# JosefAlbers/Phi-3-Vision-MLX

Measured on AMD Instinct MI355X. Metric: decode tokens/sec through generate()'s loop (reference-defined; bare graph replays: device_rate) + prefill ms, Phi-3-Vision bf16 1-image VQA, higher is better.
Workload: dtype bf16; 1 GPU; Phi-3-Vision single 336x336 image VQA (BASELINE configs[1]); 17 crops, 2509 image tokens + 22 text tokens, prompt 2531, B=1 per GPU, greedy, EOS suppressed; parallelism=batch-sharded replicas x1, batch_per_gpu=1, tiny=False

## Files before the change

include/p3v.h:

```cpp
#ifndef P3V_H
#define P3V_H
#include <stdint.h>

#ifdef __cplusplus
extern "C" {
#endif

#define P3V_VERSION 600
#define P3V_OK 0
#define P3V_ERR_ARG (-22)
#define P3V_ERR_LAUNCH (-5)
#define P3V_ERR_UNSUPPORTED (-95)
#define P3V_ERR_HIP (-14)

typedef struct {
  int cu_count, lds_per_cu, wave_size, clock_khz, mem_clock_khz, mem_bus_bits;
  int64_t hbm_bytes;
  char arch[32];
} p3v_props_t;

int p3v_version(void);
int p3v_device_props(int device, p3v_props_t* out );
const char* p3v_strerror(int code);

// ... 38 lines not shown
int p3v_gemm_rows_slices(int M, int N, int K, int epilogue);

typedef struct {
  const uint16_t* x;
  const uint16_t* W;
  void* out;
  const uint16_t* resid;
  const uint16_t* norm_w;
  float norm_eps;
  int M, N, K;
  int epilogue;
} p3v_gemv_args_t;
int p3v_gemv(const p3v_gemv_args_t* args , void* stream);

typedef struct {
  const uint16_t* x; const uint8_t* W; const float* w_scale; void* out;
  const uint16_t* resid; const uint16_t* norm_w;
  float norm_eps;
  int M, N, K;
  int epilogue;
} p3v_gemv_fp8_args_t;
int p3v_gemv_fp8(const p3v_gemv_fp8_args_t* args , void* stream);
int p3v_dequant_fp8(const uint8_t* w8, const float* w_scale, uint16_t* out_bf16, int rows, int K, void* stream);

typedef struct {
  const uint8_t* A; const float* a_scale; const uint8_t* W; const float* w_scale;
  uint16_t* out; const uint16_t* resid;
  int M, N, K, lda, ldw, ldo, epilogue;
} p3v_gemm_fp8_args_t;
int p3v_gemm_fp8(const p3v_gemm_fp8_args_t* args , void* stream);
int p3v_quant_fp8_rows(const uint16_t* x, const uint16_t* norm_w , float eps, uint8_t* q, float* scale,
                       int rows, int K, void* stream);

int p3v_rope_table(const float* pos, const float* inv_freq, float scale, float* cos_out, float* sin_out,
                   int n_pos, int half_dim, void* stream);

int p3v_rope_kv_append(const uint16_t* qkv, const float* cos_t, const float* sin_t,
                       uint16_t* q_out, uint16_t* k_dst, uint16_t* v_dst,
                       int B, int L, int n_heads, int n_kv, int hd,
                       int past, const int32_t* d_past, int dst_t, int dst_off_is_past,
                       int tab_t, int tab_div, float q_scale, void* stream);

int p3v_gemm_resid_norm(const p3v_gemm_args_t* gemm , const uint16_t* norm_w, float eps, uint16_t* normed, void* stream);

typedef struct {
  const float* cos_t; const float* sin_t;
// ... 104 lines not shown
                     int epilogue, const uint16_t* resid, uint16_t* out, int M, int N, int K, int r_max, int n_slots,
                     void* stream);

int p3v_add_i32(int32_t* x, int n, int delta, void* stream);
int p3v_store_token(const int32_t* tok, int32_t* history, const int32_t* d_step, int32_t* tok_next,
                    int B, int max_steps, void* stream);
int p3v_step_begin(const int32_t* tok, const uint16_t* table, uint16_t* x_out, const float* cos_t, const float* sin_t,
                   const int32_t* d_past, float* cos_out, float* sin_out, int B, int hidden, int vocab, int tab_t,
                   int half_dim, int32_t* zero_buf ,
                   int n_zero, void* stream);
int p3v_step_end(const uint16_t* logits, int32_t* next_tok, int32_t* tok, int32_t* history, int32_t* d_step,
                 int32_t* d_past, int32_t* ticket, int B, int n, int max_steps, void* stream);

#define P3V_GEMV_STEP_MAX_WG 1024
#define P3V_GEMV_STEP_WS_BYTES (P3V_GEMV_STEP_MAX_WG * 8 + 9 * 128)
typedef struct {
  const int32_t* tok; const uint16_t* embed_table; int vocab; uint16_t* x_out;
  const float* cos_t; const float* sin_t; float* cos_out; float* sin_out; int tab_t, half_dim;
  int32_t* next_tok; int32_t* tok_out; int32_t* history; int32_t* d_step; int32_t* ticket; float* amax_ws; int max_steps;
  int32_t* d_past;
} p3v_gemv_step_t;
int p3v_gemv_step(const p3v_gemv_args_t* args , const p3v_gemv_step_t* step , void* stream);
int p3v_gemv_fp8_step(const p3v_gemv_fp8_args_t* args , const p3v_gemv_step_t* step , void* stream);
int p3v_gemv_q4_step(const p3v_gemv_q4_args_t* args , const p3v_gemv_step_t* step , void* stream);

typedef struct {
  float temperature;
  int32_t top_k;
  float top_p;
  uint32_t seed_lo, seed_hi;
  int32_t counter;
} p3v_sample_row_t;
int p3v_sample(const uint16_t* logits, int64_t row_stride, p3v_sample_row_t* rows_params, int32_t* out, int rows, int n,
               void* stream);
int p3v_sample_step_end(const uint16_t* logits, p3v_sample_row_t* rows_params, int32_t* next_tok, int32_t* tok,
                        int32_t* history, int32_t* d_step, int32_t* d_past, int32_t* ticket, int B, int n, int max_steps,
                        void* stream);

#define P3V_LOGPROBS_MAX 8
typedef struct {
  int32_t token;
  float   logprob;
  int32_t rank;
  int32_t n_top;
  int32_t top_id[P3V_LOGPROBS_MAX];
  float   top_logprob[P3V_LOGPROBS_MAX];
// ... 53 lines not shown
```

phi-3-vision-mlx_amd/_lib.py:

```python
import ctypes as C
import os

_HERE = os.path.dirname(os.path.abspath(__file__))
LIB_PATH = os.environ.get("P3V_LIB") or os.path.join(_HERE, "libp3v.so")

P3V_OK = 0
(EPI_NONE, EPI_BIAS, EPI_BIAS_QGELU, EPI_BIAS_GELU, EPI_BIAS_RESID_F32, EPI_RESID_BF16, EPI_SILU_MUL, EPI_PATCH,
 EPI_F32) = range(9)
DECODE_MAX_L = 16

vp, i32, i64, f32 = C.c_void_p, C.c_int, C.c_int64, C.c_float


class Props(C.Structure):
    _fields_ = [("cu_count", i32), ("lds_per_cu", i32), ("wave_size", i32), ("clock_khz", i32),
                ("mem_clock_khz", i32), ("mem_bus_bits", i32), ("hbm_bytes", i64), ("arch", C.c_char * 32)]


class GemmArgs(C.Structure):
    _fields_ = [("A", vp), ("W", vp), ("out", vp), ("bias", vp), ("resid", vp), ("pos", vp),
                ("M", i32), ("N", i32), ("K", i32), ("lda", i32), ("ldw", i32), ("ldo", i32),
                ("epilogue", i32), ("patches_per_img", i32), ("ws", vp), ("ws_bytes", i64)]


# ... 1 lines not shown
    _fields_ = [("cos_t", vp), ("sin_t", vp), ("q_out", vp), ("k_dst", vp), ("v_dst", vp),
                ("B", i32), ("L", i32), ("n_heads", i32), ("n_kv", i32), ("hd", i32),
                ("past", i32), ("dst_t", i32), ("dst_off_is_past", i32), ("tab_t", i32), ("tab_div", i32), ("q_scale", f32)]


class GemvArgs(C.Structure):
    _fields_ = [("x", vp), ("W", vp), ("out", vp), ("resid", vp), ("norm_w", vp), ("norm_eps", f32),
                ("M", i32), ("N", i32), ("K", i32), ("epilogue", i32)]


class GemvStep(C.Structure):
    _fields_ = [("tok", vp), ("embed_table", vp), ("vocab", i32), ("x_out", vp),
                ("cos_t", vp), ("sin_t", vp), ("cos_out", vp), ("sin_out", vp), ("tab_t", i32), ("half_dim", i32),
                ("next_tok", vp), ("tok_out", vp), ("history", vp), ("d_step", vp), ("ticket", vp), ("amax_ws", vp), ("max_steps", i32),
                ("d_past", vp)]


GEMV_STEP_WS_BYTES = 1024 * 8 + 9 * 128


class GemvF8Args(C.Structure):
    _fields_ = [("x", vp), ("W", vp), ("w_scale", vp), ("out", vp), ("resid", vp), ("norm_w", vp), ("norm_eps", f32),
                ("M", i32), ("N", i32), ("K", i32), ("epilogue", i32)]


class GemmF8Args(C.Structure):
    _fields_ = [("A", vp), ("a_scale", vp), ("W", vp), ("w_scale", vp), ("out", vp), ("resid", vp),
                ("M", i32), ("N", i32), ("K", i32), ("lda", i32), ("ldw", i32), ("ldo", i32), ("epilogue", i32)]


class AttnArgs(C.Structure):
    _fields_ = [("q", vp), ("k_past", vp), ("v_past", vp), ("k_new", vp), ("v_new", vp), ("out", vp),
                ("pad_len", vp), ("d_past", vp), ("ws", vp),
                ("B", i32), ("L", i32), ("n_heads", i32), ("n_kv", i32), ("hd", i32),
                ("past", i32), ("past_t", i32), ("past_div", i32), ("new_t", i32), ("pad_div", i32),
                ("causal", i32), ("scale", f32), ("n_split", i32), ("new_is_cache", i32), ("q_prescaled", i32)]


class GemvQ4Args(C.Structure):
    _fields_ = [("x", vp), ("W", vp), ("sb", vp), ("out", vp), ("resid", vp), ("norm_w", vp), ("norm_eps", f32),
                ("M", i32), ("N", i32), ("K", i32), ("epilogue", i32)]


class AttnDecArgs(C.Structure):
    _fields_ = [("qkv", vp), ("cos_t", vp), ("sin_t", vp), ("k_cache", vp), ("v_cache", vp), ("out", vp),
                ("pad_len", vp), ("d_past", vp), ("ws", vp),
# ... 43 lines not shown
SPEC_REC_INTS, SPEC_CTL_INTS, SPEC_NGRAM_CAP = 18, 8, 8
SPEC_CTL_N, SPEC_CTL_NDRAFT, SPEC_CTL_FORCED, SPEC_CTL_REPLAY, SPEC_CTL_NLIMIT, SPEC_CTL_ACC = range(6)
KV_COPY_MAX_JOBS = 4
LORA_SLICE_K, LORA_MAX_RANK = 256, 64
SAMPLE_MAX_N, SAMPLE_MAX_ROWS = 32768, 1024
SIGNATURES = {
    "p3v_version": (i32, []),
    "p3v_device_props": (i32, [i32, C.POINTER(Props)]),
    "p3v_strerror": (C.c_char_p, [i32]),
    "p3v_set_tuning": (i32, [C.c_char_p, i32]),
    "p3v_get_tuning": (i32, [C.c_char_p, C.POINTER(i32)]),
    "p3v_embed_gather": (i32, [vp, vp, vp, i32, i32, i32, vp]),
    "p3v_rmsnorm": (i32, [vp, vp, vp, i32, i32, f32, vp]),
    "p3v_layernorm": (i32, [vp, vp, vp, vp, i32, i32, i32, f32, vp]),
    "p3v_gemm": (i32, [C.POINTER(GemmArgs), vp]),
    "p3v_gemm_ws_bytes": (i64, [i32, i32, i32, i32]),
    "p3v_gemm_rows_slices": (i32, [i32, i32, i32, i32]),
    "p3v_gemv": (i32, [C.POINTER(GemvArgs), vp]),
    "p3v_gemv_step": (i32, [C.POINTER(GemvArgs), C.POINTER(GemvStep), vp]),
    "p3v_gemv_fp8_step": (i32, [C.POINTER(GemvF8Args), C.POINTER(GemvStep), vp]),
    "p3v_gemv_q4_step": (i32, [C.POINTER(GemvQ4Args), C.POINTER(GemvStep), vp]),
    "p3v_gemv_fp8": (i32, [C.POINTER(GemvF8Args), vp]),
    "p3v_dequant_fp8": (i32, [vp, vp, vp, i32, i32, vp]),
    "p3v_gemm_fp8": (i32, [C.POINTER(GemmF8Args), vp]),
    "p3v_quant_fp8_rows": (i32, [vp, vp, f32, vp, vp, i32, i32, vp]),
    "p3v_rope_table": (i32, [vp, vp, f32, vp, vp, i32, i32, vp]),
    "p3v_rope_kv_append": (i32, [vp, vp, vp, vp, vp, vp, i32, i32, i32, i32, i32, i32, vp, i32, i32, i32, i32, f32, vp]),
    "p3v_attention": (i32, [C.POINTER(AttnArgs), vp]),
    "p3v_attention_decode": (i32, [C.POINTER(AttnDecArgs), vp]),
    "p3v_attention_decode_can_fuse_oproj": (i32, [i32, i32, i32, i32, i32, i32, i32, i32]),
    "p3v_attention_decode_fused_role": (i32, [i32, i32, i32, i32, i32, C.POINTER(i32)]),
    "p3v_kv_quantize": (i32, [vp, vp, vp, vp, vp, vp, i32, i32, i32, i32, i32, i32, vp]),
    "p3v_kv_dequantize": (i32, [vp, vp, vp, vp, vp, vp, i32, i32, i32, i32, i32, vp]),
    "p3v_gemm_qkv": (i32, [vp, vp, vp]),
    "p3v_gemm_resid_norm": (i32, [C.POINTER(GemmArgs), vp, f32, vp, vp]),
    "p3v_kv_quantize_mlx4": (i32, [vp, vp, vp, vp, vp, vp, i32, i32, i32, i32, vp, vp, vp, i32, i32, i32, i32, i32, vp]),
    "p3v_attention_decode_q8": (i32, [C.POINTER(AttnDecQ8Args), vp]),
    "p3v_attention_decode_q8_can_fuse_oproj": (i32, [i32, i32, i32, i32, i32, i32, i32, i32]),
    "p3v_stage_rope": (i32, [vp, vp, i32, vp, vp, vp, i32, i32, i32, i32, vp]),
    "p3v_attention_ws_bytes": (i64, [i32, i32, i32, i32, i32]),
    "p3v_im2col_patches": (i32, [vp, vp, i32, i32, i32, i32, vp]),
    "p3v_clip_cls_rows": (i32, [vp, vp, vp, i32, i32, i32, vp]),
    "p3v_hd_merge": (i32, [vp, vp, vp, vp, i32, i32, i32, i32, vp]),
    "p3v_argmax": (i32, [vp, vp, i32, i32, i64, vp]),
    "p3v_log_softmax": (i32, [vp, vp, i32, i32, vp]),
    "p3v_topk": (i32, [vp, vp, i32, i32, i32, i64, vp]),
# ... 58 lines not shown
```

phi-3-vision-mlx_amd/model.py:

```python
import math
import copy
import os

import numpy as np
import torch

from . import ops
from .config import head_dim, is_vision, rope_scaling_factor
from .weights import Q4Weight, mlx_quantize, q4_repack
from .ops import (BF16, EPI_BIAS, EPI_BIAS_GELU, EPI_BIAS_QGELU, EPI_BIAS_RESID_F32, EPI_NONE, EPI_PATCH,
                  EPI_RESID_BF16, EPI_SILU_MUL, F32, I32)

import functools
import weakref


def _on_device(fn):
    @functools.wraps(fn)
    def wrapped(self, *a, **kw):
        with torch.cuda.device(self.device):
            return fn(self, *a, **kw)
    return wrapped


# ... 123 lines not shown
        self.w8 = {}
        self._rope_tables = {}
        self._vit_graphs, self._vit_seen = {}, {}
        self.adapters = {}
        self._lora_tmp = {}
        self._lora_flat = None
        self.adapter_names = []
        self._bank = {}
        self._bank_keep = []
        self._rows_cur = None
        self.serving = os.environ.get("P3V_SHARED_GPU", "0") == "1"
        self.epoch = 0
        self._prefill_graphs = {}
        self._prefill_seen = {}
        self._states = weakref.WeakSet()
        self.fp8_act = bool(getattr(cfg, "fp8_activations", True)) and os.environ.get("P3V_FP8_PREFILL", "mfma") != "dequant"
        if getattr(cfg, "quantized_fp8", False):
            self._quantize_decoder_fp8()
        if getattr(cfg, "quantized_int4", False):
            self._quantize_decoder_q4()
        if self.w4 and not hasattr(self, "_deq"):
            n_max = max(v[0].shape[0] * v[0].shape[1] * 8 for v in self.w4.values())
            self._deq = torch.empty(n_max, dtype=BF16, device=self.device)
        if self.vision:
            self._prep_vision()

    def _quantize_decoder_fp8(self):
        names = [k for k in self.w if k == "lm_head.weight" or (k.startswith("model.layers.") and k.endswith("_proj.weight"))]
        for k in names:
            self.w8[k] = ops.quantize_fp8_rows(self.w.pop(k))
        n_max = max(v[0].shape[0] * v[0].shape[1] for v in self.w8.values())
        self._deq = torch.empty(n_max, dtype=BF16, device=self.device)

    def set_adapters(self, adapters):
        if adapters and self._bank:
            raise ValueError("this model carries an adapter bank (set_adapter_bank): detach it before set_adapters -- one or the other")
        self._set_adapters(adapters)

    @_on_device
    def _set_adapters(self, adapters):
        for k, (a, b, _) in adapters.items():
            shape = self._weight_shape(k)
            if tuple(a.shape[:1]) != (shape[1],) or tuple(b.shape[1:]) != (shape[0],):
                raise ValueError(f"LoRA shapes {tuple(a.shape)} x {tuple(b.shape)} do not fit {k} {tuple(shape)}")
        self.adapters = {k: (a.to(self.device, F32).contiguous(), b.to(self.device, F32).contiguous(), float(s))
                         for k, (a, b, s) in adapters.items()}
        self.epoch += 1
        for st in list(self._states):
            st.graphs.clear()
        self._lora_tmp, self._lora_flat = {}, None
        self._prefill_graphs.clear()

    def _weight_shape(self, k):
        if k in self.w:
            return tuple(self.w[k].shape)
# ... 95 lines not shown
        for k in names:
            self.w4[k] = tuple(t.to(self.device) for t in q4_repack(*mlx_quantize(self.w.pop(k))))

    def _proj(self, x, key, epilogue=EPI_NONE, resid=None, norm_w=None, out=None, h=None):
        ad = self.adapters.get(key)
        if ad is None:
            bk = self._bank.get(key) if self._bank else None
            if bk is not None:
                return self._proj_bank(x, key, bk[0], bk[1], epilogue, resid, norm_w, out, h)
            return self._proj_frozen(x, key, epilogue, resid, norm_w, out, h)
        a, b, scale = ad
        M, K, N, r = x.shape[0], x.shape[1], b.shape[1], a.shape[1]
        hbuf, y, t = self._lora_scratch(M, [("h", (M, K), BF16), ("y", (M, N), BF16), ("t", (M, r), F32)])
        if norm_w is not None:
            x = ops.rmsnorm(x, norm_w, self.cfg.rms_norm_eps, out=hbuf)
        self._proj_frozen(x, key, EPI_NONE, None, None, y, None)
        ops.lora_down(x, a, out=t)
        return ops.lora_up(y, t, b, scale, epilogue, resid=resid, out=out)

    def _proj_frozen(self, x, key, epilogue=EPI_NONE, resid=None, norm_w=None, out=None, h=None):
        eps = self.cfg.rms_norm_eps
        M, K = x.shape
        q, q4 = self.w8.get(key), self.w4.get(key)
        skinny = M <= 8 or (M <= ops.GEMV_MAX_M and K % 512 == 0)
        if skinny and M > 8 and q is None and q4 is None and K % 64 == 0 and self.w[key].shape[0] % 64 == 0:
            skinny = False
        if q4 is not None and M == 1 and K in (3072, 8192):
            return ops.gemv_q4(x, q4[0], q4[1], epilogue, resid=resid, norm_w=norm_w, norm_eps=eps, out=out)
        if (q4 is not None and 2 <= M <= 16 and K in (3072, 8192) and os.environ.get("P3V_Q4_ROWS", "1") != "0"
                and (q4[0].shape[0] // (2 if epilogue == EPI_SILU_MUL else 1)) % 16 == 0):
            if norm_w is not None and (M > 8 or os.environ.get("P3V_Q4_ROWS8_NORM", "1") == "0"):
                x, norm_w = ops.rmsnorm(x, norm_w, eps, out=h), None
            return ops.gemv_q4(x, q4[0], q4[1], epilogue, resid=resid, norm_w=norm_w, norm_eps=eps, out=out)
        if q is not None and skinny and K in (3072, 8192):
            return ops.gemv_fp8(x, q[0], q[1], epilogue, resid=resid, norm_w=norm_w, norm_eps=eps, out=out)
        if q is not None and not skinny and self.fp8_act and ops.gemm_fp8_ok(M, q[0].shape[0], K, epilogue):
            a8, sa = ops.quant_fp8_rows(x, norm_w, eps)
            return ops.gemm_fp8(a8, sa, q[0], q[1], epilogue, resid=resid, out=out)
        if q4 is not None:
            w = ops.dequant_q4(q4[0], q4[1], out=self._deq[:q4[0].numel() * 8].view(q4[0].shape[0], q4[0].shape[1] * 8))
        elif q is not None:
            w = ops.dequant_fp8(q[0], q[1], out=self._deq[:q[0].numel()].view(q[0].shape))
        else:
            w = self.w[key]
        if skinny:
            return ops.gemv(x, w, epilogue, resid=resid, norm_w=norm_w, norm_eps=eps, out=out)
# ... 383 lines not shown
        if (st.quantized or mlx4) and n_beam > 1:
            raise NotImplementedError("Beam Search is not yet compatible with Quantized Cache")
        mlx4_first = mlx4 and past == 0 and st.mlx4_tokens == 0 and L <= st.k4.shape[3]
        if n_beam > 1:
            Lp = (L + 7) // 8 * 8
            k_new = torch.empty((B, nkv, Lp, hd), dtype=BF16, device=self.device)
            v_new = torch.zeros((B, nkv, hd, Lp), dtype=BF16, device=self.device)
        normed_in = False
        for i in range(cfg.num_hidden_layers):
            p = f"model.layers.{i}."
            fused_qkv = False
            k_w = p + "self_attn.qkv_proj.weight"
            if (not decode and n_beam == 1 and k_w in w and k_w not in self.adapters and k_w not in self._bank and not mlx4_first
                    and (M >= 1024 or M <= 256) and os.environ.get("P3V_QKV_FUSE", "1") != "0"):
                kd, vd = (st.k_tmp, st.v_tmp) if st.quantized else (st.k[i], st.v[i])
                if not (st.quantized and past > 0 and not st.fresh_rows):
                    hn = h if normed_in else ops.rmsnorm(x, w[p + "input_layernorm.weight"], eps, out=h)
                    normed_in = True
                    fused_qkv = ops.gemm_qkv(hn, w[k_w], st.cos, st.sin, q, kd, vd, B, L, nh, nkv, hd, past, st.Tp, True, st.T, 1,
                                             q_scale=scale * ops.Q_PRESCALE)
            if i == 0 and step_begin is not None:
                sb = step_begin
                w_fold = w.get(k_w) if k_w in w else (self.w8.get(k_w) or self.w4.get(k_w))
                if not (w_fold is not None and k_w not in self.adapters and k_w not in self._bank and os.environ.get("P3V_STEP_FOLD", "1") != "0"
                        and ops.gemv_step_begin(sb["tok"], sb["table"], x, st.cos, st.sin, d_past, sb["cos_o"], sb["sin_o"],
                                                w_fold, w[p + "input_layernorm.weight"], eps, qkv)):
                    ops.step_begin(sb["tok"], sb["table"], x, st.cos, st.sin, d_past, sb["cos_o"], sb["sin_o"])
                    self._proj(x, k_w, norm_w=w[p + "input_layernorm.weight"], out=qkv, h=h)
            elif not fused_qkv:
                if normed_in:
                    self._proj(h, p + "self_attn.qkv_proj.weight", out=qkv)
                else:
                    self._proj(x, p + "self_attn.qkv_proj.weight", norm_w=w[p + "input_layernorm.weight"], out=qkv, h=h)
            o_i = o
            if fuse_o:
                o_i, o_other = (bufs["o_f"], bufs["o_f2"]) if i % 2 == 0 else (bufs["o_f2"], bufs["o_f"])
            if st.quantized:
                if decode:
                    kw_o = {}
                    if fuse_o:
                        w8o = self.w8[p + "self_attn.o_proj.weight"]
                        kw_o = dict(o_proj_w8=w8o[0], o_proj_scale=w8o[1], o_proj_x=x, o_rearm=o_other)
                    ops.attention_decode_q8(qkv, rc, rs, rb, st.k8[i], st.v8[i], st.ks[i], st.vs[i], o_i, B, L, nh, nkv,
                                            hd, scale, past, st.Tp, ws, n_split, pad_len=st.pad_len, d_past=d_past,
                                            merge_in_launch=attn_merge, **kw_o)
                else:
# ... 66 lines not shown
    def _build_decode_graph(self, st):
        cfg, B, dev = self.cfg, st.B, self.device
        g = dict(tok=torch.zeros((B,), dtype=I32, device=dev), d_past=torch.zeros((1,), dtype=I32, device=dev),
                 d_step=torch.zeros((1,), dtype=I32, device=dev),
                 history=torch.zeros((B, max(1, st.max_tokens) + 1), dtype=I32).pin_memory(),
                 x=torch.empty((B, cfg.hidden_size), dtype=BF16, device=dev),
                 logits=torch.empty((B, cfg.vocab_size), dtype=BF16, device=dev),
                 next_tok=torch.zeros((B,), dtype=I32, device=dev), ticket=torch.zeros((1,), dtype=I32, device=dev))
        g["bufs"] = self._plan(st, B, 1, fuse_o=not st.slots, captured=True)
        g["amax_ws"] = torch.zeros((ops.L.GEMV_STEP_WS_BYTES // 4,), dtype=F32, device=dev)
        g["d_past"].fill_(st.offset)
        g["gemm_ws"] = {}
        g["graph"] = self._capture(lambda: self._decode_step(st, g), g["gemm_ws"])
        g["d_step"].zero_()
        return g

    def _decode_step(self, st, g, sampled=False, logprobs=False):
        cfg, w, bufs, head = self.cfg, self.w, g["bufs"], "lm_head.weight"
        self._layers(g["x"], st, st.B, 1, 0, 1, bufs=bufs, d_past=g["d_past"],
                     step_begin=dict(tok=g["tok"], table=w["model.embed_tokens.weight"], cos_o=bufs["rope_cos"], sin_o=bufs["rope_sin"]))
        end = (g["next_tok"], g["tok"], g["history"], g["d_step"], g["d_past"], g["ticket"])
        if not sampled:
            w_fold = w.get(head) if head in w else (self.w8.get(head) or self.w4.get(head))
            if (w_fold is not None and head not in self.adapters and os.environ.get("P3V_STEP_FOLD", "1") != "0"
                    and ops.gemv_step_end(g["x"], w_fold, w["model.norm.weight"], cfg.rms_norm_eps, g["logits"], *end, g["amax_ws"])):
                return self._logprobs_tail(st, g) if logprobs else None
        self._proj(g["x"], head, norm_w=w["model.norm.weight"], out=g["logits"], h=bufs["h"])
        if sampled:
            ops.sample_step_end(g["logits"], st.sample_rows, *end)
        else:
            ops.step_end(g["logits"], *end)
        if logprobs:
            self._logprobs_tail(st, g)

    def _logprobs_tail(self, st, g):
        ops.logprobs_step(g["logits"], g["next_tok"], st.logprob_want, g["d_step"], g["records"])

    def _replay(self, token, cache, which):
        st = cache[0].state
        if st.offset + 1 > st.T:
            raise ValueError(f"KV cache overflow: {st.offset}+1 > {st.T} (prompt + max_tokens)")
        g = self._greedy_capture(st)
        if g["host_tok"] is None or token is not g["host_tok"]:
            g["tok"].copy_(token.reshape(-1).to(self.device, I32))
        if g.get("synced_offset") != st.offset:
            g["d_past"].fill_(st.offset)
# ... 328 lines not shown
```

phi-3-vision-mlx_amd/ops.py:

```python
import contextlib
import ctypes as C

import numpy as np
import torch

from . import _lib as L
from ._lib import (EPI_BIAS, EPI_BIAS_GELU, EPI_BIAS_QGELU, EPI_BIAS_RESID_F32, EPI_F32, EPI_NONE,
                   EPI_PATCH, EPI_RESID_BF16, EPI_SILU_MUL)

BF16, F32, I32 = torch.bfloat16, torch.float32, torch.int32


def _stream():
    return torch.cuda.current_stream().cuda_stream


def _p(t):
    return 0 if t is None else t.data_ptr()


def _chk(t, dtype, name):
    if not t.is_cuda:
        raise RuntimeError(f"{name}: expected a device tensor (the hot path has no CPU fallback)")
    if t.dtype != dtype:
# ... 227 lines not shown
    _chk(w4, I32, "w4"), _chk(sb, I32, "sb")
    N, K = w4.shape[0], w4.shape[1] * 8
    if out is None:
        out = torch.empty((N, K), dtype=BF16, device=w4.device)
    L.check(L.lib().p3v_dequant_q4(_p(w4), _p(sb), _p(out), N, K, _stream()), "dequant_q4")
    return out


def quantize_fp8_rows(w):
    wf = w.float()
    scale = (wf.abs().amax(dim=1) / 448.0).clamp_min(1e-12)
    w8 = (wf / scale[:, None]).to(torch.float8_e4m3fn).view(torch.uint8).contiguous()
    return w8, scale.contiguous()


def gemv_fp8(x, w8, w_scale, epilogue=EPI_NONE, resid=None, norm_w=None, norm_eps=0.0, out=None):
    _chk(x, BF16, "x"), _chk(w8, torch.uint8, "w8"), _chk(w_scale, F32, "w_scale")
    M, K = x.shape
    N = w8.shape[0] // 2 if epilogue == EPI_SILU_MUL else w8.shape[0]
    if out is None:
        out = torch.empty((M, N), dtype=F32 if epilogue == EPI_F32 else BF16, device=x.device)
    args = L.GemvF8Args(_p(x), _p(w8), _p(w_scale), _p(out), _p(resid), _p(norm_w), float(norm_eps), M, N, K, epilogue)
    L.check(L.lib().p3v_gemv_fp8(C.byref(args), _stream()), "gemv_fp8")
    return out


def dequant_fp8(w8, w_scale, out=None):
    N, K = w8.shape
    out = torch.empty((N, K), dtype=BF16, device=w8.device) if out is None else out
    L.check(L.lib().p3v_dequant_fp8(_p(w8), _p(w_scale), _p(out), N, K, _stream()), "dequant_fp8")
    return out


def quant_fp8_rows(x, norm_w=None, norm_eps=0.0, out=None, scale=None):
    _chk(x, BF16, "x")
    M, K = x.shape
    out = torch.empty((M, K), dtype=torch.uint8, device=x.device) if out is None else out
    scale = torch.empty((M,), dtype=F32, device=x.device) if scale is None else scale
    L.check(L.lib().p3v_quant_fp8_rows(_p(x), _p(norm_w), float(norm_eps), _p(out), _p(scale), M, K, _stream()), "quant_fp8_rows")
    return out, scale


def gemm_fp8(a8, a_scale, w8, w_scale, epilogue=EPI_NONE, resid=None, out=None):
    _chk(a8, torch.uint8, "a8"), _chk(w8, torch.uint8, "w8"), _chk(a_scale, F32, "a_scale"), _chk(w_scale, F32, "w_scale")
    M, K = a8.shape
    N = w8.shape[0] // 2 if epilogue == EPI_SILU_MUL else w8.shape[0]
# ... 216 lines not shown


def log_softmax(x):
    _chk(x, BF16, "x")
    n = x.shape[-1]
    y = torch.empty_like(x)
    L.check(L.lib().p3v_log_softmax(_p(x), _p(y), x.numel() // n, n, _stream()), "log_softmax")
    return y


def topk(x2d, k):
    _chk(x2d, BF16, "x")
    rows, n = x2d.shape
    out = torch.empty((rows, k), dtype=I32, device=x2d.device)
    L.check(L.lib().p3v_topk(_p(x2d), _p(out), rows, n, k, n, _stream()), "topk")
    return out


def gemv_step_begin(tok, table, x_out, cos_t, sin_t, d_past, cos_out, sin_out, w, norm_w, norm_eps, out):
    _chk(table, BF16, "table"), _chk(x_out, BF16, "x_out"), _chk(tok, I32, "tok")
    B, tab_t, half = tok.numel(), cos_t.shape[-2], cos_t.shape[-1]
    st = L.GemvStep(_p(tok), _p(table), table.shape[0], _p(x_out), _p(cos_t), _p(sin_t), _p(cos_out), _p(sin_out), tab_t, half,
                    None, None, None, None, None, None, 0, _p(d_past))
    if isinstance(w, tuple) and w[0].dtype == I32:
        w4, sb = w
        _chk(sb, I32, "sb")
        args = L.GemvQ4Args(None, _p(w4), _p(sb), _p(out), None, _p(norm_w), float(norm_eps), B, w4.shape[0], w4.shape[1] * 8, EPI_NONE)
        rc = L.lib().p3v_gemv_q4_step(C.byref(args), C.byref(st), _stream())
    elif isinstance(w, tuple):
        w8, ws = w
        _chk(w8, torch.uint8, "w8"), _chk(ws, F32, "w_scale")
        args = L.GemvF8Args(None, _p(w8), _p(ws), _p(out), None, _p(norm_w), float(norm_eps), B, w8.shape[0], w8.shape[1], EPI_NONE)
        rc = L.lib().p3v_gemv_fp8_step(C.byref(args), C.byref(st), _stream())
    else:
        _chk(w, BF16, "w")
        args = L.GemvArgs(None, _p(w), _p(out), None, _p(norm_w), float(norm_eps), B, w.shape[0], w.shape[1], EPI_NONE)
        rc = L.lib().p3v_gemv_step(C.byref(args), C.byref(st), _stream())
    if rc == L.ERR_UNSUPPORTED:
        return False
    L.check(rc, "gemv_step(begin)")
    return True


def gemv_step_end(x, w, norm_w, norm_eps, out, next_tok, tok, history, d_step, d_past, ticket, amax_ws):
    _chk(x, BF16, "x"), _chk(out, BF16, "out")
    if amax_ws.numel() * amax_ws.element_size() < L.GEMV_STEP_WS_BYTES:
        raise ValueError("gemv_step_end: amax_ws smaller than P3V_GEMV_STEP_WS_BYTES")
    M, K = x.shape
    st = L.GemvStep(None, None, 0, None, None, None, None, None, 0, 0,
                    _p(next_tok), _p(tok), _p(history), _p(d_step), _p(ticket), _p(amax_ws), history.shape[1], _p(d_past))
    if isinstance(w, tuple) and w[0].dtype == I32:
        w4, sb = w
        _chk(sb, I32, "sb")
        args = L.GemvQ4Args(_p(x), _p(w4), _p(sb), _p(out), None, _p(norm_w), float(norm_eps), M, w4.shape[0], K, EPI_NONE)
        rc = L.lib().p3v_gemv_q4_step(C.byref(args), C.byref(st), _stream())
    elif isinstance(w, tuple):
        w8, ws = w
        _chk(w8, torch.uint8, "w8"), _chk(ws, F32, "w_scale")
        args = L.GemvF8Args(_p(x), _p(w8), _p(ws), _p(out), None, _p(norm_w), float(norm_eps), M, w8.shape[0], K, EPI_NONE)
        rc = L.lib().p3v_gemv_fp8_step(C.byref(args), C.byref(st), _stream())
    else:
        _chk(w, BF16, "w")
        args = L.GemvArgs(_p(x), _p(w), _p(out), None, _p(norm_w), float(norm_eps), M, w.shape[0], K, EPI_NONE)
        rc = L.lib().p3v_gemv_step(C.byref(args), C.byref(st), _stream())
    if rc == L.ERR_UNSUPPORTED:
        return False
    L.check(rc, "gemv_step(end)")
    return True


def add_i32(x, delta):
    L.check(L.lib().p3v_add_i32(_p(x), x.numel(), int(delta), _stream()), "add_i32")


# ... 161 lines not shown
```

Measured before the change: 534.3 tokens/s.

## Pack decoder bf16 weights losslessly into 13-bit format for decode GEMVs

Adds a lossless 13-bit weight format: 1 sign bit, 7 mantissa bits and a 5-bit exponent offset from a per-matrix base. It is applied when a matrix's exponent range fits in 31 values, and is used for the qkv, gate_up, down and lm_head M=1 decode GEMVs, including the fused step-begin and step-end kernels. Weight reads bound the decode loop, so cutting weight bytes by about a fifth should lower HBM traffic per token. The cost is extra in-register decode work using perm and packed u16 ops, a one-time pack at load, and extra memory held by keeping both copies. Matrices whose exponents don't fit fall back to the existing paths.

```diff
diff --git a/include/p3v.h b/include/p3v.h
--- a/include/p3v.h
+++ b/include/p3v.h
@@ -84,6 +84,18 @@
 } p3v_gemv_fp8_args_t;
 int p3v_gemv_fp8(const p3v_gemv_fp8_args_t* args , void* stream);
 int p3v_dequant_fp8(const uint8_t* w8, const float* w_scale, uint16_t* out_bf16, int rows, int K, void* stream);
+
+int p3v_pack_b13(const uint16_t* W, int rows, int K, int silu_pairs, void* out, int32_t* info, void* stream);
+int p3v_unpack_b13(const void* packed, int rows, int K, int silu_pairs, int exp_base, uint16_t* out_bf16, void* stream);
+typedef struct {
+  const uint16_t* x; const void* W; void* out;
+  const uint16_t* resid; const uint16_t* norm_w;
+  float norm_eps;
+  int M, N, K;
+  int epilogue;
+  int exp_base, silu_pairs;
+} p3v_gemv_b13_args_t;
+int p3v_gemv_b13(const p3v_gemv_b13_args_t* args , void* stream);
 
 typedef struct {
   const uint8_t* A; const float* a_scale; const uint8_t* W; const float* w_scale;
@@ -234,6 +246,7 @@
 } p3v_gemv_step_t;
 int p3v_gemv_step(const p3v_gemv_args_t* args , const p3v_gemv_step_t* step , void* stream);
 int p3v_gemv_fp8_step(const p3v_gemv_fp8_args_t* args , const p3v_gemv_step_t* step , void* stream);
+int p3v_gemv_b13_step(const p3v_gemv_b13_args_t* args , const p3v_gemv_step_t* step , void* stream);
 int p3v_gemv_q4_step(const p3v_gemv_q4_args_t* args , const p3v_gemv_step_t* step , void* stream);
 
 typedef struct {
diff --git a/phi-3-vision-mlx_amd/_lib.py b/phi-3-vision-mlx_amd/_lib.py
--- a/phi-3-vision-mlx_amd/_lib.py
+++ b/phi-3-vision-mlx_amd/_lib.py
@@ -47,6 +47,11 @@
 class GemvF8Args(C.Structure):
     _fields_ = [("x", vp), ("W", vp), ("w_scale", vp), ("out", vp), ("resid", vp), ("norm_w", vp), ("norm_eps", f32),
                 ("M", i32), ("N", i32), ("K", i32), ("epilogue", i32)]
+
+
+class GemvB13Args(C.Structure):
+    _fields_ = [("x", vp), ("W", vp), ("out", vp), ("resid", vp), ("norm_w", vp), ("norm_eps", f32),
+                ("M", i32), ("N", i32), ("K", i32), ("epilogue", i32), ("exp_base", i32), ("silu_pairs", i32)]
 
 
 class GemmF8Args(C.Structure):
@@ -136,6 +141,10 @@
     "p3v_gemv_q4_step": (i32, [C.POINTER(GemvQ4Args), C.POINTER(GemvStep), vp]),
     "p3v_gemv_fp8": (i32, [C.POINTER(GemvF8Args), vp]),
     "p3v_dequant_fp8": (i32, [vp, vp, vp, i32, i32, vp]),
+    "p3v_pack_b13": (i32, [vp, i32, i32, i32, vp, vp, vp]),
+    "p3v_unpack_b13": (i32, [vp, i32, i32, i32, i32, vp, vp]),
+    "p3v_gemv_b13": (i32, [C.POINTER(GemvB13Args), vp]),
+    "p3v_gemv_b13_step": (i32, [C.POINTER(GemvB13Args), C.POINTER(GemvStep), vp]),
     "p3v_gemm_fp8": (i32, [C.POINTER(GemmF8Args), vp]),
     "p3v_quant_fp8_rows": (i32, [vp, vp, f32, vp, vp, i32, i32, vp]),
     "p3v_rope_table": (i32, [vp, vp, f32, vp, vp, i32, i32, vp]),
diff --git a/phi-3-vision-mlx_amd/csrc/p3v_dot_b13.h b/phi-3-vision-mlx_amd/csrc/p3v_dot_b13.h
--- /dev/null
+++ b/phi-3-vision-mlx_amd/csrc/p3v_dot_b13.h
@@ -0,0 +1,29 @@
+#pragma once
+#include "p3v_common.h"
+
+template <int CH> struct B13 {
+  static_assert(CH == 4 || CH == 6, "a container is 26 or 39 dwords per lane");
+  static constexpr int D = 13 * CH / 2, NS = D - 6 * CH;
+  static constexpr int NIB_OFF = 64 * NS, LO_OFF = NIB_OFF + (CH / 2) * 256, DWORDS = 64 * D;
+  static __host__ __device__ constexpr int sign_word(int row, int j, int half) { return (row * 2 * CH + 2 * j + half) >> 3; }
+  static __host__ __device__ constexpr int sign_shift(int row, int j, int half) { return (row * 2 * CH + 2 * j + half) & 7; }
+};
+
+typedef unsigned short b13_u16x2_t __attribute__((ext_vector_type(2)));
+
+__device__ __forceinline__ u32x4_t b13_decode8(uint32_t lo0, uint32_t lo1, uint32_t nib, uint32_t sg0, uint32_t sg1, uint32_t cc) {
+  const uint32_t hi0 = (sg0 & 0x80808080u) | (nib & 0x0f0f0f0fu), hi1 = (sg1 & 0x80808080u) | ((nib >> 4) & 0x0f0f0f0fu);
+  const uint32_t pre[4] = {__builtin_amdgcn_perm(hi0, lo0, 0x05010400u), __builtin_amdgcn_perm(hi0, lo0, 0x07030602u),
+                           __builtin_amdgcn_perm(hi1, lo1, 0x05010400u), __builtin_amdgcn_perm(hi1, lo1, 0x07030602u)};
+  const b13_u16x2_t c2 = __builtin_bit_cast(b13_u16x2_t, cc), one = {1, 1}, mag = {0x7fff, 0x7fff};
+  u32x4_t w;
+#pragma unroll
+  for (int d = 0; d < 4; ++d) {
+    const b13_u16x2_t p = __builtin_bit_cast(b13_u16x2_t, pre[d]);
+    b13_u16x2_t n, r;
+    asm("v_pk_min_u16 %0, %1, %2" : "=v"(n) : "v"(p & mag), "v"(one));
+    asm("v_pk_mad_u16 %0, %1, %2, %3" : "=v"(r) : "v"(n), "v"(c2), "v"(p));
+    w[d] = __builtin_bit_cast(uint32_t, r);
+  }
+  return w;
+}
diff --git a/phi-3-vision-mlx_amd/csrc/p3v_gemv_b13.hip b/phi-3-vision-mlx_amd/csrc/p3v_gemv_b13.hip
--- /dev/null
+++ b/phi-3-vision-mlx_amd/csrc/p3v_gemv_b13.hip
@@ -0,0 +1,213 @@
+#include <type_traits>
+
+#include "p3v_common.h"
+#include "p3v_dot_b13.h"
+#include "p3v_dot_bf16.h"
+#include "p3v_gemv3_body.h"
+
+struct GemvB13P {
+  const bf16_t* x; const uint32_t* W; void* out; const bf16_t* resid; const bf16_t* norm_w;
+  float eps;
+  int M, N, K, epi, units;
+  uint32_t cc;
+};
+
+struct GemvB13 {
+  typedef GemvB13P P;
+  static constexpr int WPL = 8, MAX_MT = 1;
+  static constexpr bool XSUM = false;
+  template <int CH> struct Stage { uint32_t sg[B13<CH>::NS]; u32x4_t nib[CH / 2]; u32x4_t lo[CH]; uint32_t cc; };
+  static int wpc() { return p3v_tuning().gemv_wpc; }
+  static __device__ __forceinline__ void mark(int) {}
+  template <int K, int CH>
+  static __device__ __forceinline__ void load(const P& p, int r0, int, int c0, Stage<CH>& st) {
+    typedef B13<CH> L;
+    constexpr int NST = K / (CH * 512);
+    const int u = p.epi == P3V_EPI_SILU_MUL ? r0 : r0 >> 1, lane = c0 & 63, s = (c0 >> 6) / CH;
+    const uint32_t* cp = p.W + (size_t)(u * NST + s) * L::DWORDS;
+    if constexpr (L::NS == 3) {
+      const uint32_t* sp = cp + lane * 3;
+      st.sg[0] = __builtin_nontemporal_load(sp);
+      st.sg[1] = __builtin_nontemporal_load(sp + 1);
+      st.sg[2] = __builtin_nontemporal_load(sp + 2);
+    } else {
+      const u32x2_t v = __builtin_nontemporal_load((const u32x2_t*)cp + lane);
+      st.sg[0] = v[0];
+      st.sg[1] = v[1];
+    }
+    const u32x4_t* np = (const u32x4_t*)(cp + L::NIB_OFF) + lane;
+    const u32x4_t* lp = (const u32x4_t*)(cp + L::LO_OFF) + lane;
+#pragma unroll
+    for (int i = 0; i < CH / 2; ++i) st.nib[i] = __builtin_nontemporal_load(np + i * 64);
+#pragma unroll
+    for (int j = 0; j < CH; ++j) st.lo[j] = __builtin_nontemporal_load(lp + j * 64);
+    st.cc = p.cc;
+  }
+  template <int CH>
+  static __device__ __forceinline__ u32x4_t weights(const Stage<CH>& st, int j, int row) {
+    typedef B13<CH> L;
+    return b13_decode8(st.lo[j][2 * row], st.lo[j][2 * row + 1], st.nib[j >> 1][(j & 1) * 2 + row],
+                       st.sg[L::sign_word(row, j, 0)] << L::sign_shift(row, j, 0), st.sg[L::sign_word(row, j, 1)] << L::sign_shift(row, j, 1), st.cc);
+  }
+  template <int CH>
+  static __device__ __forceinline__ void dot(const Stage<CH>& st, int j, const u32x4_t* x, const float*, int c, float& a0, float& a1) {
+    const u32x4_t xa = x[c];
+    a0 = dot8(weights(st, j, 0), xa, a0);
+    a1 = dot8(weights(st, j, 1), xa, a1);
+  }
+  template <int CH> static __device__ __forceinline__ float finish(float v, const Stage<CH>&, int) { return v; }
+};
+
+#define B13_BAD_VALUE 1
+#define B13_BAD_RANGE 2
+
+__global__ void k_b13_init(int32_t* info) { info[0] = 0; info[1] = 1; info[2] = 255; info[3] = 0; }
+
+__global__ void __launch_bounds__(256) k_b13_range(const u32x4_t* __restrict__ W, long chunks, int32_t* info) {
+  int emin = 255, emax = 0, bad = 0;
+  for (long i = (long)blockIdx.x * 256 + threadIdx.x; i < chunks; i += (long)gridDim.x * 256) {
+    const u32x4_t w = W[i];
+#pragma unroll
+    for (int k = 0; k < 8; ++k) {
+      const uint32_t h = (w[k >> 1] >> (16 * (k & 1))) & 0xffffu, e = (h >> 7) & 0xffu, m = h & 0x7fu;
+      if (e == 255u || (e == 0u && m != 0u)) bad = 1;
+      if (e != 0u) { emin = min(emin, (int)e); emax = max(emax, (int)e); }
+    }
+  }
+#pragma unroll
+  for (int off = 32; off > 0; off >>= 1) {
+    emin = min(emin, __shfl_xor(emin, off, 64));
+    emax = max(emax, __shfl_xor(emax, off, 64));
+    bad |= __shfl_xor(bad, off, 64);
+  }
+  if ((threadIdx.x & 63) == 0) {
+    atomicMin(info + 2, emin);
+    atomicMax(info + 3, emax);
+    if (bad) atomicOr(info, B13_BAD_VALUE);
+  }
+}
+
+template <int CH>
+__global__ void __launch_bounds__(256) k_b13_pack(const u32x4_t* __restrict__ W, uint32_t* __restrict__ out, int32_t* info, int rows, int nst,
+                                                  int silu_pairs, long n_lanes) {
+  typedef B13<CH> L;
+  const int emin = info[2], emax = info[3];
+  const int base = max(1, emax - 30);
+  const long t = (long)blockIdx.x * 256 + threadIdx.x;
+  if (t == 0) {
+    info[1] = base;
+    if (emin < base) atomicOr(info, B13_BAD_RANGE);
+  }
+  if (t >= n_lanes || emin < base) return;
+  const long ci = t >> 6;
+  const int lane = (int)(t & 63), u = (int)(ci / nst), s = (int)(ci % nst), xch = nst * CH * 64;
+  const int r[2] = {silu_pairs ? u : 2 * u, silu_pairs ? u + rows / 2 : 2 * u + 1};
+  uint32_t sg[L::NS] = {};
+  u32x4_t nib[CH / 2], lo[CH];
+#pragma unroll
+  for (int i = 0; i < CH / 2; ++i) nib[i] = (u32x4_t){0, 0, 0, 0};
+#pragma unroll
+  for (int j = 0; j < CH; ++j) lo[j] = (u32x4_t){0, 0, 0, 0};
+#pragma unroll
+  for (int row = 0; row < 2; ++row)
+#pragma unroll
+    for (int j = 0; j < CH; ++j) {
+      const u32x4_t w = W[(size_t)r[row] * xch + (s * CH + j) * 64 + lane];
+#pragma unroll
+      for (int k = 0; k < 8; ++k) {
+        const uint32_t h = (w[k >> 1] >> (16 * (k & 1))) & 0xffffu, e = (h >> 7) & 0xffu, m = h & 0x7fu, sign = h >> 15;
+        const uint32_t q = e == 0u ? 0u : (e - (uint32_t)base + 1u) & 31u;
+        const int half = k >> 2, b = k & 3;
+        lo[j][2 * row + half] |= (((q & 1u) << 7) | m) << (8 * b);
+        nib[j >> 1][(j & 1) * 2 + row] |= (q >> 1) << (4 * (2 * b + half));
+        sg[L::sign_word(row, j, half)] |= sign << (8 * b + 7 - L::sign_shift(row, j, half));
+      }
+    }
+  uint32_t* cp = out + (size_t)ci * L::DWORDS;
+#pragma unroll
+  for (int i = 0; i < L::NS; ++i) cp[lane * L::NS + i] = sg[i];
+#pragma unroll
+  for (int i = 0; i < CH / 2; ++i) ((u32x4_t*)(cp + L::NIB_OFF))[i * 64 + lane] = nib[i];
+#pragma unroll
+  for (int j = 0; j < CH; ++j) ((u32x4_t*)(cp + L::LO_OFF))[j * 64 + lane] = lo[j];
+}
+
+template <int K, int CH>
+__global__ void __launch_bounds__(256) k_b13_unpack(GemvB13P p, u32x4_t* __restrict__ out, int rows, long n_lanes) {
+  constexpr int NST = K / (CH * 512);
+  const long t = (long)blockIdx.x * 256 + threadIdx.x;
+  if (t >= n_lanes) return;
+  const long ci = t >> 6;
+  const int lane = (int)(t & 63), u = (int)(ci / NST), s = (int)(ci % NST);
+  const bool silu = p.epi == P3V_EPI_SILU_MUL;
+  const int r[2] = {silu ? u : 2 * u, silu ? u + rows / 2 : 2 * u + 1};
+  GemvB13::Stage<CH> st;
+  GemvB13::load<K, CH>(p, r[0], r[1], s * CH * 64 + lane, st);
+#pragma unroll
+  for (int row = 0; row < 2; ++row)
+#pragma unroll
+    for (int j = 0; j < CH; ++j) out[(size_t)r[row] * (K / 8) + (s * CH + j) * 64 + lane] = GemvB13::weights(st, j, row);
+}
+
+static bool b13_shape_ok(int rows, int K) { return rows > 0 && rows % 2 == 0 && (K == 3072 || K == 8192); }
+static uint32_t b13_cc(int base) { const uint32_t c = (uint32_t)(base - 1) << 7; return c | (c << 16); }
+
+extern "C" int p3v_pack_b13(const uint16_t* W, int rows, int K, int silu_pairs, void* out, int32_t* info, void* stream) {
+  if (!W || !out || !info) return P3V_ERR_ARG;
+  if (!b13_shape_ok(rows, K)) return P3V_ERR_UNSUPPORTED;
+  if (((uintptr_t)W | (uintptr_t)out) & 15) return P3V_ERR_ARG;
+  hipStream_t s = (hipStream_t)stream;
+  const long chunks = (long)rows * (K / 8), n_lanes = chunks / (K == 3072 ? 12 : 8);
+  hipLaunchKernelGGL(k_b13_init, dim3(1), dim3(1), 0, s, info);
+  hipLaunchKernelGGL(k_b13_range, dim3(min(4096, p3v_cdiv(chunks, 256))), dim3(256), 0, s, (const u32x4_t*)W, chunks, info);
+  if (K == 3072) hipLaunchKernelGGL(k_b13_pack<6>, dim3(p3v_cdiv(n_lanes, 256)), dim3(256), 0, s, (const u32x4_t*)W, (uint32_t*)out, info, rows, 1, silu_pairs, n_lanes);
+  else hipLaunchKernelGGL(k_b13_pack<4>, dim3(p3v_cdiv(n_lanes, 256)), dim3(256), 0, s, (const u32x4_t*)W, (uint32_t*)out, info, rows, 4, silu_pairs, n_lanes);
+  P3V_CHECK_LAUNCH();
+  return P3V_OK;
+}
+
+extern "C" int p3v_unpack_b13(const void* packed, int rows, int K, int silu_pairs, int exp_base, uint16_t* out, void* stream) {
+  if (!packed || !out || exp_base < 1 || exp_base > 224) return P3V_ERR_ARG;
+  if (!b13_shape_ok(rows, K)) return P3V_ERR_UNSUPPORTED;
+  if (((uintptr_t)packed | (uintptr_t)out) & 15) return P3V_ERR_ARG;
+  GemvB13P p = {nullptr, (const uint32_t*)packed, nullptr, nullptr, nullptr, 0.f, 1, rows, K, silu_pairs ? P3V_EPI_SILU_MUL : P3V_EPI_NONE, rows / 2, b13_cc(exp_base)};
+  const long n_lanes = (long)rows * (K / 8) / (K == 3072 ? 12 : 8);
+  hipStream_t s = (hipStream_t)stream;
+  if (K == 3072) hipLaunchKernelGGL((k_b13_unpack<3072, 6>), dim3(p3v_cdiv(n_lanes, 256)), dim3(256), 0, s, p, (u32x4_t*)out, rows, n_lanes);
+  else hipLaunchKernelGGL((k_b13_unpack<8192, 4>), dim3(p3v_cdiv(n_lanes, 256)), dim3(256), 0, s, p, (u32x4_t*)out, rows, n_lanes);
+  P3V_CHECK_LAUNCH();
+  return P3V_OK;
+}
+
+static int b13_params(const p3v_gemv_b13_args_t* a, GemvB13P& p) {
+  if (a->M <= 0 || a->N <= 0) return P3V_ERR_ARG;
+  if (a->M != 1 || a->N % 2 || (a->K != 3072 && a->K != 8192)) return P3V_ERR_UNSUPPORTED;
+  if (a->exp_base < 1 || a->exp_base > 224 || ((uintptr_t)a->W & 15)) return P3V_ERR_ARG;
+  if ((a->silu_pairs != 0) != (a->epilogue == P3V_EPI_SILU_MUL)) return P3V_ERR_ARG;
+  p = {a->x, (const uint32_t*)a->W, a->out, a->resid, a->norm_w, a->norm_eps, a->M, a->N, a->K, a->epilogue,
+       a->epilogue == P3V_EPI_SILU_MUL ? a->N : a->N / 2, b13_cc(a->exp_base)};
+  return P3V_OK;
+}
+
+extern "C" int p3v_gemv_b13_step(const p3v_gemv_b13_args_t* a, const p3v_gemv_step_t* st, void* stream) {
+  if (!a || !st || !a->W || !a->out) return P3V_ERR_ARG;
+  GemvStepP sp; bool begin;
+  if (const int rc = gemv_step_params(a, st, true, sp, begin)) return rc;
+  GemvB13P p;
+  if (const int rc = b13_params(a, p)) return rc;
+  hipStream_t s = (hipStream_t)stream;
+  if (a->K == 3072) return begin ? launch_gemv_stream<GemvB13, 1, 1, 6, STEP_BEGIN>(p, s, &sp) : launch_gemv_stream<GemvB13, 1, 1, 6, STEP_END>(p, s, &sp);
+  return begin ? launch_gemv_stream<GemvB13, 1, 4, 4, STEP_BEGIN>(p, s, &sp) : launch_gemv_stream<GemvB13, 1, 4, 4, STEP_END>(p, s, &sp);
+}
+
+extern "C" int p3v_gemv_b13(const p3v_gemv_b13_args_t* a, void* stream) {
+  if (!a || !a->x || !a->W || !a->out) return P3V_ERR_ARG;
+  if (a->epilogue != P3V_EPI_NONE && a->epilogue != P3V_EPI_RESID_BF16 && a->epilogue != P3V_EPI_SILU_MUL &&
+      a->epilogue != P3V_EPI_F32)
+    return P3V_ERR_UNSUPPORTED;
+  if (a->epilogue == P3V_EPI_RESID_BF16 && !a->resid) return P3V_ERR_ARG;
+  GemvB13P p;
+  if (const int rc = b13_params(a, p)) return rc;
+  hipStream_t s = (hipStream_t)stream;
+  return a->K == 3072 ? launch_gemv_stream<GemvB13, 1, 1, 6>(p, s) : launch_gemv_stream<GemvB13, 1, 4, 4>(p, s);
+}
diff --git a/phi-3-vision-mlx_amd/model.py b/phi-3-vision-mlx_amd/model.py
--- a/phi-3-vision-mlx_amd/model.py
+++ b/phi-3-vision-mlx_amd/model.py
@@ -169,6 +169,9 @@
         if self.w4 and not hasattr(self, "_deq"):
             n_max = max(v[0].shape[0] * v[0].shape[1] * 8 for v in self.w4.values())
             self._deq = torch.empty(n_max, dtype=BF16, device=self.device)
+        self.w13 = {}
+        if os.environ.get("P3V_PACK13", "1") != "0":
+            self._pack_decoder_b13()
         if self.vision:
             self._prep_vision()
 
@@ -178,6 +181,33 @@
             self.w8[k] = ops.quantize_fp8_rows(self.w.pop(k))
         n_max = max(v[0].shape[0] * v[0].shape[1] for v in self.w8.values())
         self._deq = torch.empty(n_max, dtype=BF16, device=self.device)
+
+    @_on_device
+    def _pack_decoder_b13(self):
+        for k, v in self.w.items():
+            if k != "lm_head.weight" and not (k.startswith("model.layers.") and k.endswith(("qkv_proj.weight", "gate_up_proj.weight", "down_proj.weight"))):
+                continue
+            if v.dim() != 2 or v.shape[1] not in (3072, 8192) or v.shape[0] % 2:
+                continue
+            pk = ops.pack_b13(v, silu_pairs=k.endswith("gate_up_proj.weight"))
+            if pk is not None:
+                self.w13[k] = pk
+
+    def _packed(self, key):
+        pk = self.w13.get(key)
+        if pk is not None and not pk.current(self.w.get(key)):
+            del self.w13[key]
+            self.epoch += 1
+            return None
+        return pk
+
+    def repack_b13(self):
+        self.w13.clear()
+        self.epoch += 1
+        for st in list(self._states):
+            st.graphs.clear()
+        if os.environ.get("P3V_PACK13", "1") != "0":
+            self._pack_decoder_b13()
 
     def set_adapters(self, adapters):
         if adapters and self._bank:
@@ -319,6 +349,9 @@
         eps = self.cfg.rms_norm_eps
         M, K = x.shape
         q, q4 = self.w8.get(key), self.w4.get(key)
+        pk = self._packed(key) if M == 1 else None
+        if pk is not None and pk.silu_pairs == (epilogue == EPI_SILU_MUL):
+            return ops.gemv_b13(x, pk, epilogue, resid=resid, norm_w=norm_w, norm_eps=eps, out=out)
         skinny = M <= 8 or (M <= ops.GEMV_MAX_M and K % 512 == 0)
         if skinny and M > 8 and q is None and q4 is None and K % 64 == 0 and self.w[key].shape[0] % 64 == 0:
             skinny = False
@@ -748,6 +781,8 @@
             if i == 0 and step_begin is not None:
                 sb = step_begin
                 w_fold = w.get(k_w) if k_w in w else (self.w8.get(k_w) or self.w4.get(k_w))
+                if B == 1 and self._packed(k_w) is not None:
+                    w_fold = self.w13[k_w]
                 if not (w_fold is not None and k_w not in self.adapters and k_w not in self._bank and os.environ.get("P3V_STEP_FOLD", "1") != "0"
                         and ops.gemv_step_begin(sb["tok"], sb["table"], x, st.cos, st.sin, d_past, sb["cos_o"], sb["sin_o"],
                                                 w_fold, w[p + "input_layernorm.weight"], eps, qkv)):
@@ -860,6 +895,8 @@
         end = (g["next_tok"], g["tok"], g["history"], g["d_step"], g["d_past"], g["ticket"])
         if not sampled:
             w_fold = w.get(head) if head in w else (self.w8.get(head) or self.w4.get(head))
+            if st.B == 1 and self._packed(head) is not None:
+                w_fold = self.w13[head]
             if (w_fold is not None and head not in self.adapters and os.environ.get("P3V_STEP_FOLD", "1") != "0"
                     and ops.gemv_step_end(g["x"], w_fold, w["model.norm.weight"], cfg.rms_norm_eps, g["logits"], *end, g["amax_ws"])):
                 return self._logprobs_tail(st, g) if logprobs else None
diff --git a/phi-3-vision-mlx_amd/ops.py b/phi-3-vision-mlx_amd/ops.py
--- a/phi-3-vision-mlx_amd/ops.py
+++ b/phi-3-vision-mlx_amd/ops.py
@@ -1,5 +1,6 @@
 import contextlib
 import ctypes as C
+import weakref
 
 import numpy as np
 import torch
@@ -273,6 +274,52 @@
         out = torch.empty((M, N), dtype=F32 if epilogue == EPI_F32 else BF16, device=x.device)
     args = L.GemvF8Args(_p(x), _p(w8), _p(w_scale), _p(out), _p(resid), _p(norm_w), float(norm_eps), M, N, K, epilogue)
     L.check(L.lib().p3v_gemv_fp8(C.byref(args), _stream()), "gemv_fp8")
+    return out
+
+
+class PackedB13:
+    __slots__ = ("data", "base", "rows", "K", "silu_pairs", "src", "version")
+
+    def __init__(self, data, base, rows, K, silu_pairs, src=None):
+        self.data, self.base, self.rows, self.K, self.silu_pairs = data, int(base), int(rows), int(K), bool(silu_pairs)
+        self.src, self.version = (weakref.ref(src) if src is not None else None), (src._version if src is not None else 0)
+
+    def current(self, w):
+        return w is not None and self.src is not None and w is self.src() and w._version == self.version
+
+
+def pack_b13(w, silu_pairs=False):
+    _chk(w, BF16, "w")
+    rows, K = w.shape
+    if K not in (3072, 8192) or rows % 2:
+        return None
+    data = torch.empty((rows, K * 13 // 8), dtype=torch.uint8, device=w.device)
+    info = torch.empty(4, dtype=I32, device=w.device)
+    L.check(L.lib().p3v_pack_b13(_p(w), rows, K, int(bool(silu_pairs)), _p(data), _p(info), _stream()), "pack_b13")
+    status, base = info.tolist()[:2]
+    return None if status else PackedB13(data, base, rows, K, silu_pairs, src=w)
+
+
+def unpack_b13(pk, out=None):
+    out = torch.empty((pk.rows, pk.K), dtype=BF16, device=pk.data.device) if out is None else out
+    L.check(L.lib().p3v_unpack_b13(_p(pk.data), pk.rows, pk.K, int(pk.silu_pairs), pk.base, _p(out), _stream()), "unpack_b13")
+    return out
+
+
+def _b13_args(x, pk, out, resid, norm_w, norm_eps, M, epilogue):
+    N = pk.rows // 2 if epilogue == EPI_SILU_MUL else pk.rows
+    return L.GemvB13Args(_p(x), _p(pk.data), _p(out), _p(resid), _p(norm_w), float(norm_eps), M, N, pk.K, epilogue, pk.base, int(pk.silu_pairs))
+
+
+def gemv_b13(x, pk, epilogue=EPI_NONE, resid=None, norm_w=None, norm_eps=0.0, out=None):
+    _chk(x, BF16, "x")
+    M, K = x.shape
+    if K != pk.K:
+        raise ValueError(f"gemv_b13: x has {K} columns, the packed matrix {pk.K}")
+    if out is None:
+        out = torch.empty((M, pk.rows // 2 if epilogue == EPI_SILU_MUL else pk.rows), dtype=F32 if epilogue == EPI_F32 else BF16, device=x.device)
+    args = _b13_args(x, pk, out, resid, norm_w, norm_eps, M, epilogue)
+    L.check(L.lib().p3v_gemv_b13(C.byref(args), _stream()), "gemv_b13")
     return out
 
 
@@ -535,7 +582,12 @@
     B, tab_t, half = tok.numel(), cos_t.shape[-2], cos_t.shape[-1]
     st = L.GemvStep(_p(tok), _p(table), table.shape[0], _p(x_out), _p(cos_t), _p(sin_t), _p(cos_out), _p(sin_out), tab_t, half,
                     None, None, None, None, None, None, 0, _p(d_past))
-    if isinstance(w, tuple) and w[0].dtype == I32:
+    if isinstance(w, PackedB13):
+        if table.shape[1] != w.K or x_out.shape[-1] != w.K:
+            raise ValueError(f"gemv_step_begin: table / x_out rows of {table.shape[1]} / {x_out.shape[-1]} columns, the packed matrix {w.K}")
+        args = _b13_args(None, w, out, None, norm_w, norm_eps, B, EPI_NONE)
+        rc = L.lib().p3v_gemv_b13_step(C.byref(args), C.byref(st), _stream())
+    elif isinstance(w, tuple) and w[0].dtype == I32:
         w4, sb = w
         _chk(sb, I32, "sb")
         args = L.GemvQ4Args(None, _p(w4), _p(sb), _p(out), None, _p(norm_w), float(norm_eps), B, w4.shape[0], w4.shape[1] * 8, EPI_NONE)
@@ -562,7 +614,12 @@
     M, K = x.shape
     st = L.GemvStep(None, None, 0, None, None, None, None, None, 0, 0,
                     _p(next_tok), _p(tok), _p(history), _p(d_step), _p(ticket), _p(amax_ws), history.shape[1], _p(d_past))
-    if isinstance(w, tuple) and w[0].dtype == I32:
+    if isinstance(w, PackedB13):
+        if K != w.K:
+            raise ValueError(f"gemv_step_end: x has {K} columns, the packed matrix {w.K}")
+        args = _b13_args(x, w, out, None, norm_w, norm_eps, M, EPI_NONE)
+        rc = L.lib().p3v_gemv_b13_step(C.byref(args), C.byref(st), _stream())
+    elif isinstance(w, tuple) and w[0].dtype == I32:
         w4, sb = w
         _chk(sb, I32, "sb")
         args = L.GemvQ4Args(_p(x), _p(w4), _p(sb), _p(out), None, _p(norm_w), float(norm_eps), M, w4.shape[0], K, EPI_NONE)
```

After: 555.9 tokens/s, median of 6. 1.04x the previous value.
